# SEEDtk/kmers.anno

Hardware: AMD Instinct MI355X
Metric: kmer lookups/s + seqs annotated/s at 1/2/4/8 GPUs; achieved HBM GB/s vs roofline (higher is better)
Workload: dtype u64; 1 GPU; c5: 1M proteins per rank vs 10^8-entry multi-function signature table (HBM random access); proteins_per_gpu=1000000, windows_per_gpu=303576763, batch_windows=303576763, table_entries=100000000, functions=100000, k=8, min_hits=5, table_layout_m=6, table_minimizer_order=mod-sampling, table_placement=two-choice, parallelism=input-shard x1, table on this GPU

## Files before the change

kmers.anno_amd/csrc/kma_abi.cpp:

```cpp
#include <hip/hip_runtime.h>
#include <sched.h>

#include <algorithm>
#include <atomic>
#include <chrono>
#include <condition_variable>
#include <cstdarg>
#include <cstdio>
#include <cstdlib>
#include <cstring>
#include <memory>
#include <mutex>
#include <string>
#include <thread>
#include <vector>

#include "../../include/kmeranno.h"
#include "kma_distance.h"
#include "kma_hashanno.h"
#include "kma_internal.h"
#include "kma_pack.h"
#include "kma_tsv.h"

namespace {
// ... 1200 lines not shown
uint64_t contig_blocks(uint64_t n_bases) {
  return std::max<uint64_t>(1, (n_bases + kma::kContigTile - 1) / kma::kContigTile);
}

void codon_codes(const char* code, uint8_t out[64]) {
  for (int i = 0; i < 64; ++i)
    out[i] = (code[i] == '*' || code[i] == 'X') ? 0 : (uint8_t)(code[i] - 'A' + 1);
}

int contig_args(const kma_table* t, const Replica& r, kma_workspace* ws, const uint8_t* d_dna,
                const uint64_t* d_offsets, uint32_t n_contig, uint64_t n_bases, const char* code,
                uint32_t* d_tally, uint32_t n_fid, hipStream_t s, kma::ContigArgs* out) {
  kma::ContigArgs a{};
  a.slots = r.d_slots;
  a.n_buckets = (uint32_t)t->n_buckets;
  a.dna = d_dna;
  a.offsets = d_offsets;
  a.n_contig = n_contig;
  a.total_bases = n_bases;
  a.k = t->k;
  a.mlen = t->mlen;
  a.two_choice = t->two_choice ? 1u : 0u;
  a.staging = ws->d_cstage;
  a.block_counts = ws->d_ccounts;
  if (ws->cpending) KMA_HIP(hipMemsetAsync(ws->d_cprefix, 0, (ws->cgroups + 1) * 8, s));
  ws->cpending = true;
  a.group_sum = ws->d_cprefix;
  a.emit_done = reinterpret_cast<uint32_t*>(ws->d_cprefix + ws->cgroups);
  a.tally = d_tally;
  a.n_fid = d_tally ? n_fid : 0;
  codon_codes(code, a.codon_codes);
  *out = a;
  return KMA_OK;
}

int enqueue_contig_emit(kma_workspace* ws, kma::ContigArgs a, kma_hit* d_hits, uint64_t cap,
                        uint64_t* d_n_hits, hipStream_t s) {
  const uint64_t nb = contig_blocks(a.total_bases);
  a.out = d_hits;
  a.cap = d_hits ? cap : 0;
  a.n_hits = d_n_hits;
  KMA_HIP(kma::launch_contigs_emit(a, nb, s));
  ws->cpending = false;
  return KMA_OK;
}

struct PhaseClock {
  hipEvent_t* ev = nullptr;
  int n = 0;
  hipStream_t s = nullptr;
  PhaseClock(kma_workspace* ws, hipStream_t stream, const char* const* names, int n_phases)
      : s(stream) {
    if (!ws->timing) return;
    const uint32_t slot = ws->n_timed++ % kTimingRing;
    ev = &ws->events[kMaxEv * slot];
    ws->names[slot] = names;
    ws->n_phases[slot] = n_phases;
  }
  hipError_t mark() { return ev ? hipEventRecord(ev[n++], s) : hipSuccess; }
};

const char* const kDirectPhases[] = {"annotate_kernel"};
const char* const kPackedPhases[] = {"pack_kernel", "annotate_kernel"};
const char* const kContigPhases[] = {"contigs_probe_kernel", "scan_emit"};

uint32_t block_proteins(const kma_workspace* ws, uint32_t n_seq, uint64_t table_bytes) {
  const int64_t f = ws->opt_block_proteins != kOptUnset ? ws->opt_block_proteins
                                                         : opt(KMA_OPT_BLOCK_PROTEINS);
  if (f >= 1 && f <= kma::kBlockProteins) return (uint32_t)f;
  const uint64_t slots = (uint64_t)kma::kProteinOcc * (uint64_t)std::max(ws->n_cu, 1);
  return (uint64_t)n_seq / 6 > 4 * slots && table_bytes > kInfinityCacheBytes ? 6u : 4u;
}

uint32_t defer_below(const kma_workspace* ws, uint64_t n_groups) {
  const uint64_t slots = (uint64_t)kma::kProteinOcc * (uint64_t)std::max(ws->n_cu, 1);
  const int64_t f = ws->opt_defer != kOptUnset ? ws->opt_defer : opt(KMA_OPT_DEFER);
  if (f >= 0) return (uint32_t)std::min<int64_t>(64, f);
  return n_groups > slots && n_groups <= 4 * slots ? 3u : 0u;
}

enum class Input { kAscii, kPackOnDevice, kStream };

constexpr uint64_t kPackMinResidues = 1ull << 25;
bool pack_on_device(uint64_t n_residues) {
  const int64_t v = opt(KMA_OPT_PACKED_INPUT);
  return n_residues > 0 && (v == 2 || (v == 1 && n_residues >= kPackMinResidues));
}

int ensure_packed(const kma_workspace* ws) {
  if (ws->d_packed) return KMA_OK;
  return fail(KMA_E_CAPACITY, "workspace has no packed stream (kma_workspace_reserve_batch first)");
}

int annotate_proteins_on(const kma_table* t, const Replica& r, kma_workspace* ws,
                         const uint8_t* d_residues, const uint64_t* d_offsets, uint32_t n_seq,
                         uint64_t n_residues, int min_hits, uint32_t flags, int32_t* d_fid,
                         int32_t* d_count, uint8_t* d_status, uint32_t* d_tally, uint32_t n_fid,
                         hipStream_t s, Input input = Input::kAscii, uint64_t stream_first = 0) {
  kma::ProteinArgs a{};
  a.slots = r.d_slots;
  a.n_buckets = (uint32_t)t->n_buckets;
  a.lut = r.d_lut;
  a.residues = input == Input::kPackOnDevice ? ws->d_packed : d_residues;
  a.packed = input != Input::kAscii;
  a.stream_first = input == Input::kStream ? stream_first : 0;
  a.offsets = d_offsets;
  a.n_seq = n_seq;
  a.n_residues = (uint32_t)n_residues;
  a.k = t->k;
  a.mlen = t->mlen;
  a.two_choice = t->two_choice ? 1u : 0u;
  a.min_hits = min_hits;
  a.flags = flags;
  a.out_fid = d_fid;
  a.out_count = d_count;
  a.out_status = d_status;
  a.tally = d_tally;
  a.n_fid = d_tally ? n_fid : 0;
  a.gset = ws->d_gset;
  a.block_proteins = block_proteins(ws, n_seq, t->n_buckets * (uint64_t)kma::kBucketBytes);
  a.n_groups = (n_seq + a.block_proteins - 1) / a.block_proteins;
  a.defer_below = a.n_groups < (1u << 30) ? defer_below(ws, a.n_groups) : 0u;
  const bool pack = input == Input::kPackOnDevice;
  PhaseClock clk(ws, s, pack ? kPackedPhases : kDirectPhases, pack ? 2 : 1);
  KMA_HIP(clk.mark());
  if (pack) {
    KMA_HIP(kma::launch_pack_residues(d_residues, d_offsets, n_residues, r.d_lut, ws->d_packed,
                                      s));
    KMA_HIP(clk.mark());
  }
  KMA_HIP(kma::launch_annotate(a, s));
  KMA_HIP(clk.mark());
  return KMA_OK;
}

int check_protein_call(const kma_table* t, int min_hits, uint32_t flags) {
  if (!t) return fail(KMA_E_INVALID, "null table");
  if (kma::wide_k(t->k))
    return fail(KMA_E_INVALID, "the protein path takes tables of K <= 8 (this table: K = %d)",
                t->k);
  if (min_hits < 1) return fail(KMA_E_INVALID, "Min-hits must be positive.");
  if (flags & ~(KMA_F_END_EXCLUSIVE | KMA_F_MULTISET)) return fail(KMA_E_INVALID, "bad flags");
  return KMA_OK;
}

hipError_t stage_h2d(uint8_t* d_dst, uint8_t* h_pinned, const uint8_t* src, size_t len,
                     int device, hipStream_t s) {
  constexpr size_t kChunk = 2u << 20;
  const size_t n_chunks = (len + kChunk - 1) / kChunk;
  staging_pool().run(n_chunks, staging_threads(), [&](uint64_t i) {
    const size_t off = i * kChunk;
    std::memcpy(h_pinned + off, src + off, std::min(kChunk, len - off));
  });
  (void)device;
  return len ? hipMemcpyAsync(d_dst, h_pinned, len, hipMemcpyHostToDevice, s) : hipSuccess;
}

hipError_t stage_pack_h2d(uint8_t* d_stream, uint8_t* h_stream, const uint8_t* lut,
                          const uint8_t* residues, uint64_t n_res, uint64_t ga, uint64_t gb,
                          uint64_t tail, hipStream_t s) {
  constexpr uint64_t kChunkGroups = 1u << 15;
  const uint64_t n_chunks = std::max<uint64_t>(1, (gb - ga + kChunkGroups - 1) / kChunkGroups);
  staging_pool().run(n_chunks, staging_threads(), [&](uint64_t i) {
    const uint64_t g0 = ga + i * kChunkGroups, g1 = std::min(gb, g0 + kChunkGroups);
    const uint64_t r0 = 64 * g0, r1 = std::min(64 * g1, n_res);
    const uint64_t bytes = 40 * (g1 - g0) + (g1 == gb ? tail : 0);
    kma::pack_residues_host(lut, residues + r0, r1 > r0 ? r1 - r0 : 0, h_stream + 40 * g0, bytes);
  });
  const uint64_t bytes = 40 * (gb - ga) + tail;
// ... 318 lines not shown
    ws->names.assign(kTimingRing, nullptr);
    ws->n_phases.assign(kTimingRing, 0);
  }
  ws->timing = enable != 0;
  ws->n_timed = 0;
  return KMA_OK;
}

int kma_workspace_phases_read(kma_workspace* ws, uint32_t* n_calls, int* n_phases,
                              double* phase_ms, const char** phase_names) {
  if (!ws || !n_calls || !n_phases || !phase_ms) return fail(KMA_E_INVALID, "null argument");
  DeviceScope ds(ws->device);
  const uint32_t n = std::min(ws->n_timed, kTimingRing);
  *n_calls = 0;
  *n_phases = 0;
  for (int i = 0; i < KMA_MAX_PHASES; ++i) {
    phase_ms[i] = 0.0;
    if (phase_names) phase_names[i] = nullptr;
  }
  if (n == 0) return KMA_OK;
  const uint32_t last = (ws->n_timed - 1) % kTimingRing;
  const char* const* names = ws->names[last];
  const int np = ws->n_phases[last];
  for (uint32_t i = 0; i < n; ++i) {
    if (ws->names[i] != names) continue;
    hipEvent_t* e = &ws->events[kMaxEv * i];
    KMA_HIP(hipEventSynchronize(e[np]));
    for (int ph = 0; ph < np; ++ph) {
      float ms = 0;
      KMA_HIP(hipEventElapsedTime(&ms, e[ph], e[ph + 1]));
      phase_ms[ph] += ms;
    }
    ++*n_calls;
  }
  *n_phases = np;
  if (phase_names)
    for (int ph = 0; ph < np; ++ph) phase_names[ph] = names[ph];
  ws->n_timed = 0;
  return KMA_OK;
}

int kma_workspace_timing_read(kma_workspace* ws, uint32_t* n_calls, double* kernel_ms,
                              double* rest_ms) {
  if (!ws || !n_calls || !kernel_ms || !rest_ms) return fail(KMA_E_INVALID, "null argument");
  double ms[KMA_MAX_PHASES];
  const char* names[KMA_MAX_PHASES];
  int np = 0;
  if (int rc = kma_workspace_phases_read(ws, n_calls, &np, ms, names)) return rc;
  const bool contigs = np > 0 && names[0] == kContigPhases[0];
  *kernel_ms = 0;
  *rest_ms = 0;
  for (int ph = 0; ph < np; ++ph) (contigs && ph > 0 ? *rest_ms : *kernel_ms) += ms[ph];
  return KMA_OK;
}

int kma_workspace_destroy(kma_workspace* ws) {
  if (!ws) return KMA_OK;
  DeviceScope ds(ws->device);
  for (auto& e : ws->events) (void)hipEventDestroy(e);
  free_protein_scratch(ws);
  free_contig_scratch(ws);
  delete ws;
  return KMA_OK;
}

int kma_annotate_proteins_device(const kma_table* t, kma_workspace* ws, const uint8_t* d_residues,
                                 const uint64_t* d_offsets, uint32_t n_seq, uint64_t n_residues,
                                 int min_hits, uint32_t flags, int32_t* d_fid, int32_t* d_count,
                                 uint8_t* d_status, uint32_t* d_tally, uint32_t n_fid,
                                 void* stream) {
  if (int rc = check_protein_call(t, min_hits, flags)) return rc;
  if (!ws) return fail(KMA_E_INVALID, "null workspace");
  Replica rep;
  if (!replica_on(t, ws->device, &rep))
    return fail(KMA_E_INVALID, "table has no replica on the workspace's device %d", ws->device);
  const Replica* r = &rep;
  if (n_seq == 0) return KMA_OK;
  if (!d_residues || !d_offsets || !d_fid || !d_count || !d_status)
    return fail(KMA_E_INVALID, "null device buffer");
  if ((uintptr_t)d_residues & 7) return fail(KMA_E_INVALID, "residues must be 8-byte aligned");
  if (n_residues > ws->res_cap)
    return fail(KMA_E_CAPACITY, "workspace reserved for %llu residues, call needs %llu",
                (unsigned long long)ws->res_cap, (unsigned long long)n_residues);
  const bool pack = pack_on_device(n_residues);
  if (pack)
    if (int rc = ensure_packed(ws)) return rc;
  DeviceScope ds(r->device);
  if (ds.err != hipSuccess) return fail(KMA_E_DEVICE, "hipSetDevice(%d)", r->device);
  return annotate_proteins_on(t, *r, ws, d_residues, d_offsets, n_seq, n_residues, min_hits,
                              flags, d_fid, d_count, d_status, d_tally, n_fid,
                              static_cast<hipStream_t>(stream),
                              pack ? Input::kPackOnDevice : Input::kAscii);
}

uint64_t kma_packed_bytes(uint64_t n_residues) { return kma::packed_bytes(n_residues); }

int kma_pack_residues(const kma_table* t, const uint8_t* residues, uint64_t n, uint8_t* out,
                      uint64_t out_bytes) {
  if ((n && !residues) || !out) return fail(KMA_E_INVALID, "null argument");
  if (out_bytes < kma::packed_bytes(n))
    return fail(KMA_E_CAPACITY, "packed stream of %llu residues needs %llu bytes",
                (unsigned long long)n, (unsigned long long)kma::packed_bytes(n));
  uint8_t std_lut[256];
  if (!t) standard_lut(std_lut);
  const uint8_t* lut = t ? t->lut : std_lut;
  constexpr uint64_t kChunkGroups = 1u << 15;
  const uint64_t n_groups = (n + 63) / 64, n_chunks = (n_groups + kChunkGroups - 1) / kChunkGroups;
  if (n_chunks < 4) {
    kma::pack_residues_host(lut, residues, n, out, out_bytes);
    return KMA_OK;
  }
  staging_pool().run(n_chunks, staging_threads(), [&](uint64_t c) {
    const uint64_t g0 = c * kChunkGroups, g1 = std::min(n_groups, g0 + kChunkGroups);
    const uint64_t r0 = 64 * g0, r1 = std::min(64 * g1, n);
    const uint64_t bytes = g1 == n_groups ? out_bytes - 40 * g0 : 40 * (g1 - g0);
    kma::pack_residues_host(lut, residues + r0, r1 - r0, out + 40 * g0, bytes);
  });
  return KMA_OK;
}

int kma_annotate_packed_device(const kma_table* t, kma_workspace* ws, const uint8_t* d_stream,
                               const uint64_t* d_offsets, uint32_t n_seq, uint64_t n_residues,
                               int min_hits, uint32_t flags, int32_t* d_fid, int32_t* d_count,
                               uint8_t* d_status, uint32_t* d_tally, uint32_t n_fid,
                               void* stream) {
  if (int rc = check_protein_call(t, min_hits, flags)) return rc;
  if (!ws) return fail(KMA_E_INVALID, "null workspace");
  Replica rep;
  if (!replica_on(t, ws->device, &rep))
    return fail(KMA_E_INVALID, "table has no replica on the workspace's device %d", ws->device);
  if (n_seq == 0) return KMA_OK;
  if (!d_stream || !d_offsets || !d_fid || !d_count || !d_status)
    return fail(KMA_E_INVALID, "null device buffer");
  if ((uintptr_t)d_stream & 7) return fail(KMA_E_INVALID, "stream must be 8-byte aligned");
  if (n_residues > ws->res_cap)
    return fail(KMA_E_CAPACITY, "workspace reserved for %llu residues, call needs %llu",
                (unsigned long long)ws->res_cap, (unsigned long long)n_residues);
  DeviceScope ds(rep.device);
  if (ds.err != hipSuccess) return fail(KMA_E_DEVICE, "hipSetDevice(%d)", rep.device);
  return annotate_proteins_on(t, rep, ws, d_stream, d_offsets, n_seq, n_residues, min_hits, flags,
                              d_fid, d_count, d_status, d_tally, n_fid,
                              static_cast<hipStream_t>(stream), Input::kStream, 0);
}

int kma_annotate_proteins(const kma_table* tc, const uint8_t* residues, const uint64_t* offsets,
                          uint32_t n_seq, int min_hits, uint32_t flags, int32_t* out_fid,
                          int32_t* out_count, uint8_t* out_status, uint32_t* out_tally,
                          uint32_t n_fid) {
  if (int rc = check_protein_call(tc, min_hits, flags)) return rc;
  kma_table* t = const_cast<kma_table*>(tc);
  if (n_seq == 0) return KMA_OK;
  if (!residues || !offsets || !out_fid || !out_count || !out_status)
    return fail(KMA_E_INVALID, "null argument");
  if (const uint32_t s = offsets_decrease_at(offsets, n_seq); s < n_seq)
    return fail(KMA_E_INVALID, "offsets decrease at %u", s);
  const bool tally = out_tally && n_fid;
  const std::vector<Replica> reps = replicas(t);
  const int nr = (int)std::min<uint64_t>(reps.size(), n_seq);
  const std::vector<uint32_t> b = shard_bounds(offsets, n_seq, nr);
  std::vector<std::vector<uint32_t>> part(tally ? nr : 0, std::vector<uint32_t>(n_fid));
  const int64_t so = opt(KMA_OPT_HOST_SLICE);
  const uint64_t slice = so > 0 ? (uint64_t)so : 1ull << 31;
  const size_t width = staging_width(nr);
  const int rc = fan_out(nr, [&](int i) {
    ShardWidth sw(width);
    std::vector<uint32_t> st(tally ? n_fid : 0);
    for (uint32_t lo = b[i]; lo < b[i + 1];) {
// ... 793 lines not shown
```

kmers.anno_amd/csrc/kma_device.h:

```cpp
#pragma once

#include <hip/hip_runtime.h>
#include <stdint.h>

#include "kma_internal.h"

namespace kma {
namespace {

template <typename Op>
__device__ __forceinline__ uint32_t wave_reduce(uint32_t v, Op op) {
  v = op(v, (uint32_t)__builtin_amdgcn_mov_dpp((int)v, 0xB1, 0xF, 0xF, false));
  v = op(v, (uint32_t)__builtin_amdgcn_mov_dpp((int)v, 0x4E, 0xF, 0xF, false));
  v = op(v, (uint32_t)__builtin_amdgcn_mov_dpp((int)v, 0x141, 0xF, 0xF, false));
  v = op(v, (uint32_t)__builtin_amdgcn_mov_dpp((int)v, 0x140, 0xF, 0xF, false));
  const uint32_t r0 = (uint32_t)__builtin_amdgcn_readlane((int)v, 0);
  const uint32_t r1 = (uint32_t)__builtin_amdgcn_readlane((int)v, 16);
  const uint32_t r2 = (uint32_t)__builtin_amdgcn_readlane((int)v, 32);
  const uint32_t r3 = (uint32_t)__builtin_amdgcn_readlane((int)v, 48);
  return op(op(r0, r1), op(r2, r3));
}
__device__ __forceinline__ uint32_t wave_max(uint32_t v) {
  return wave_reduce(v, [](uint32_t x, uint32_t y) { return x > y ? x : y; });
}
__device__ __forceinline__ uint32_t wave_sum(uint32_t v) {
  return wave_reduce(v, [](uint32_t x, uint32_t y) { return x + y; });
}
__device__ __forceinline__ uint32_t popc_below(uint64_t m) {
  return __builtin_amdgcn_mbcnt_hi((uint32_t)(m >> 32),
                                   __builtin_amdgcn_mbcnt_lo((uint32_t)m, 0u));
}

__device__ __forceinline__ uint64_t funnel(uint64_t lo, uint64_t hi, uint32_t sh) {
  return sh ? ((lo >> sh) | (hi << (64u - sh))) : lo;
}
__device__ __forceinline__ uint64_t window_bytes(const uint8_t* __restrict__ res, uint64_t pos) {
  const uint64_t* src = reinterpret_cast<const uint64_t*>(res + (pos & ~7ull));
  return funnel(src[0], src[1], (uint32_t)(pos & 7) * 8u);
}
struct WinWords {
  uint64_t lo, hi;
  uint32_t sh;
};
__device__ __forceinline__ WinWords window_words(const uint8_t* __restrict__ res, uint64_t pos) {
  const uint64_t* src = reinterpret_cast<const uint64_t*>(res + (pos & ~7ull));
  return WinWords{src[0], src[1], (uint32_t)(pos & 7) * 8u};
}
__device__ __forceinline__ uint64_t win_bytes(const WinWords& w) { return funnel(w.lo, w.hi, w.sh); }

__device__ __forceinline__ WinWords window_words_packed(const uint8_t* __restrict__ stream,
                                                        uint64_t j) {
  const uint64_t bit = 5 * j, byte = bit >> 3;
  const uint64_t* src = reinterpret_cast<const uint64_t*>(stream + (byte & ~7ull));
  return WinWords{src[0], src[1], (uint32_t)(((byte & 7) << 3) | (bit & 7))};
}
__device__ __forceinline__ uint64_t bswap64(uint64_t v) {
  const uint32_t lo = (uint32_t)v, hi = (uint32_t)(v >> 32);
  const uint32_t slo = __builtin_amdgcn_perm(0u, lo, 0x00010203u);
  const uint32_t shi = __builtin_amdgcn_perm(0u, hi, 0x00010203u);
  return (uint64_t)slo << 32 | shi;
}
template <int K>
__device__ __forceinline__ uint64_t packed_key(const WinWords& w) {
  const uint64_t be = bswap64(funnel(w.lo, w.hi, w.sh & 56u));
  return (be << (w.sh & 7u)) >> (64 - 5 * K);
}

template <int K>
__device__ __forceinline__ bool pack_window(const uint8_t* lut, uint64_t bytes, uint64_t& key) {
  uint32_t c[K];
#pragma unroll
  for (int j = 0; j < K; ++j) c[j] = lut[(uint32_t)(bytes >> (8 * j)) & 0xFFu];
  uint64_t v = 0;
  bool ok = true;
#pragma unroll
  for (int j = 0; j < K; ++j) {
    ok = ok && c[j] != 0u;
    v = (v << 5) | c[j];
  }
  key = v;
  return ok;
}

constexpr int kBucketQuads = kBucketBytes / 16;
__device__ __forceinline__ void scan_half(const uint4 (&q)[4], int half, uint64_t key, bool& hit,
                                          bool& empty, uint32_t& fid, uint32_t& slot) {
  const uint32_t klo = (uint32_t)key, khi = (uint32_t)(key >> 32) << 24;
  const uint32_t lo[8] = {q[0].x, q[0].z, q[1].x, q[1].z, q[2].x, q[2].z, q[3].x, q[3].z};
  const uint32_t hi[8] = {q[0].y, q[0].w, q[1].y, q[1].w, q[2].y, q[2].w, q[3].y, q[3].w};
#pragma unroll
  for (int j = 0; j < 8; ++j) {
    const bool m = lo[j] == klo && (hi[j] & kKeyHiMask) == khi;
    fid = m ? (hi[j] & kFidMask) : fid;
    slot = m ? (uint32_t)(8 * half + j) : slot;
    hit = hit || m;
    empty = empty || lo[j] == 0u;
  }
}

#ifndef KMA_WALK_GROUP
#define KMA_WALK_GROUP 1
#endif
constexpr int kWalkGroup = KMA_WALK_GROUP;
__device__ __forceinline__ bool walk_chain(const uint64_t* __restrict__ slots, uint32_t n_buckets,
                                           uint32_t b, uint64_t key, uint32_t& fid,
                                           uint32_t& sid, bool two_choice = false,
                                           uint32_t* walked = nullptr) {
  if (two_choice) {
    const uint32_t ab = alt_bucket(key, b, n_buckets);
    const uint4* bp = reinterpret_cast<const uint4*>(slots + (uint64_t)ab * kSlotsPerBucket);
    uint4 q[kBucketQuads];
#pragma unroll
    for (int i = 0; i < kBucketQuads; ++i) q[i] = bp[i];
    bool h = false, e = false;
    uint32_t slot = 0;
#pragma unroll
    for (int half = 0; half < kBucketHalves; ++half) {
      const uint4 part[4] = {q[4 * half], q[4 * half + 1], q[4 * half + 2], q[4 * half + 3]};
      scan_half(part, half, key, h, e, fid, slot);
    }
    sid = ab * kSlotsPerBucket + slot;
    if (walked) *walked = 1;
    return h;
  }
  bool hit = false, empty = false;
  const uint32_t home = b;
  uint32_t slot = 0, steps = 1;
  while (!hit && !empty && steps < n_buckets) {
    uint32_t bb[kWalkGroup];
    uint4 q[kWalkGroup][kBucketQuads];
#pragma unroll
    for (int g = 0; g < kWalkGroup; ++g) {
      const uint32_t i = steps + g;
      b = chain_bucket(home, i < n_buckets ? i : 0u, n_buckets);
      bb[g] = b;
      const uint4* bp = reinterpret_cast<const uint4*>(slots + (uint64_t)b * kSlotsPerBucket);
#pragma unroll
      for (int i = 0; i < kBucketQuads; ++i) q[g][i] = bp[i];
    }
#pragma unroll
    for (int g = 0; g < kWalkGroup; ++g) {
      if (hit || empty || steps >= n_buckets) break;
      bool h = false, e = false;
#pragma unroll
      for (int half = 0; half < kBucketHalves; ++half) {
        const uint4 part[4] = {q[g][4 * half], q[g][4 * half + 1], q[g][4 * half + 2],
                               q[g][4 * half + 3]};
        scan_half(part, half, key, h, e, fid, slot);
      }
      hit = h;
      empty = e;
      sid = bb[g] * kSlotsPerBucket + slot;
      ++steps;
    }
  }
  if (walked) *walked = steps - 1;
  return hit;
}

template <int R>
__device__ __forceinline__ uint32_t quad_bcast(uint32_t v) {
  return (uint32_t)__builtin_amdgcn_mov_dpp((int)v, R * 0x55, 0xF, 0xF, false);
}
__device__ __forceinline__ uint32_t quad_or(uint32_t v) {
// ... 134 lines not shown
```

kmers.anno_amd/csrc/kma_kernels.hip:

```cpp
#include <cstring>
#include <rocprim/rocprim.hpp>

#include <algorithm>
#include <cstdio>
#include <cstdlib>

#include "../../include/kmeranno.h"
#include "kma_internal.h"
#include "kma_device.h"


namespace kma {
namespace {


template <bool Wide>
__global__ __launch_bounds__(256) void build_insert_kernel(uint64_t* slots, uint32_t* winner,
                                                           uint32_t n_buckets, int k, int m,
                                                           const uint64_t* __restrict__ keys,
                                                           uint64_t n, uint32_t* status) {
  constexpr int S = Wide ? kWideSlots : kSlotsPerBucket;
  for (uint64_t i = blockIdx.x * (uint64_t)blockDim.x + threadIdx.x; i < n;
       i += (uint64_t)gridDim.x * blockDim.x) {
    const uint64_t key = keys[i];
// ... 192 lines not shown
        if (chosen >> j & 1ull) continue;
        const uint64_t key = skeys[ids[i + j]];
        const uint32_t mask = filter_need<S>((uint32_t)key);
        const bool alt_full = load && load[alt_bucket(key, h, n_buckets)] >= S;
        const uint32_t fresh = (uint32_t)__popc(mask & ~set) + (alt_full ? 32u : 0u);
        if (fresh < best_new) {
          best = j;
          best_new = fresh;
          best_mask = mask;
          if (fresh == 0) break;
        }
      }
      chosen |= 1ull << best;
      set |= best_mask;
      away[ids[i + best]] = 1;
    }
  }
}

__global__ __launch_bounds__(256) void build_two_choice_filter_kernel(uint64_t* slots,
                                                                      uint32_t n_buckets, int k,
                                                                      int m, uint32_t* stats) {
  constexpr int S = kSlotsPerBucket;
  const uint64_t n_slots = (uint64_t)n_buckets * S;
  uint32_t entries = 0, displaced = 0;
  for (uint64_t i = blockIdx.x * (uint64_t)blockDim.x + threadIdx.x; i < n_slots;
       i += (uint64_t)gridDim.x * blockDim.x) {
    const uint64_t v = __hip_atomic_load(slots + i, __ATOMIC_RELAXED, __HIP_MEMORY_SCOPE_AGENT);
    if ((uint32_t)v == 0u) continue;
    const uint64_t key = slot_key(v);
    const uint32_t b = (uint32_t)(i / S), h = home_bucket(key, k, m, n_buckets);
    entries++;
    if (b != h) {
      displaced++;
      for (int f = 0; f < kFilterBits; ++f) {
        const uint32_t pos = filter_pos<S>((uint32_t)key, f);
        uint32_t* meta = reinterpret_cast<uint32_t*>(slots + (uint64_t)h * S + pos / kFilterBits) + 1;
        const uint32_t bit = 1u << (kFidBits + pos % kFilterBits);
        if (!(__hip_atomic_load(meta, __ATOMIC_RELAXED, __HIP_MEMORY_SCOPE_AGENT) & bit))
          atomicOr(meta, bit);
      }
    }
  }
  entries = wave_sum(entries);
  displaced = wave_sum(displaced);
  if ((threadIdx.x & 63) == 0) {
    if (entries) atomicAdd(stats + 0, entries);
    atomicMax(stats + 1, displaced ? 2u : entries ? 1u : 0u);
    if (displaced) atomicAdd(stats + 2, displaced);
  }
}


#ifdef KMA_BLOCK_CLOCK
__device__ uint64_t g_block_clk[8 * 65536];
#define KMA_CLK_SET(i, v)                                          \
  do {                                                             \
    if (threadIdx.x == 0 && blockIdx.x < 65535)                    \
      g_block_clk[8 * blockIdx.x + (i)] = (v);                     \
  } while (0)
#define KMA_CLK(i) KMA_CLK_SET(i, wall_clock64())
#define KMA_CLK_HW()                                                \
  KMA_CLK_SET(6, (uint64_t)__builtin_amdgcn_s_getreg(20 | (15 << 11)) << 32 | \
                     (uint32_t)__builtin_amdgcn_s_getreg(4 | (31 << 11)))
#else
#define KMA_CLK_SET(i, v) ((void)0)
#define KMA_CLK(i) ((void)0)
#define KMA_CLK_HW() ((void)0)
#endif

#ifdef KMA_TUNE_COUNT
__device__ unsigned long long g_walk_stats[8];
#define KMA_COUNT(i, v)                                                                    \
  do {                                                                                     \
    const unsigned long long kma_v_ = (unsigned long long)(v);   \
    if ((threadIdx.x & 63) == 0)                                                           \
      __hip_atomic_fetch_add(&g_walk_stats[i], kma_v_, __ATOMIC_RELAXED,                   \
                             __HIP_MEMORY_SCOPE_AGENT);                                    \
  } while (0)
#else
#define KMA_COUNT(i, v) ((void)0)
#endif

template <int P>
struct ProteinSmem {
  __attribute__((aligned(16))) uint32_t pool[kSetPool];
  uint32_t chain_q[kWavesPerBlock][2 * kChainQ];
  uint32_t pbeg[P + 1];
  uint32_t pwin[P];
  uint32_t pset[P];
  uint32_t pcap[P];
  uint32_t pmin[P], pmax[P], pcnt[P];
  uint32_t plist[P];
  uint32_t skip;
  uint8_t lut[256];
};
static_assert(sizeof(ProteinSmem<kBlockProteins>) <= 163840 / kProteinOcc,
              "protein-path LDS must leave kProteinOcc blocks per CU");

__device__ __forceinline__ bool lds_set_insert(uint32_t* set, uint32_t cap, uint32_t key) {
  uint32_t i = set_slot(key, cap);
  for (;;) {
    const uint32_t o = atomicCAS(set + i, 0u, key);
    if (o == 0u) return true;
    if (o == key) return false;
    i = i + 1 == cap ? 0u : i + 1;
  }
}
__device__ __forceinline__ bool global_set_insert(uint32_t* set, uint32_t cap, uint32_t key) {
  uint32_t i = set_slot(key, cap);
  for (;;) {
    uint32_t o = 0u;
    __hip_atomic_compare_exchange_strong(set + i, &o, key, __ATOMIC_RELAXED, __ATOMIC_RELAXED,
                                         __HIP_MEMORY_SCOPE_AGENT);
    if (o == 0u) return true;
    if (o == key) return false;
    i = i + 1 == cap ? 0u : i + 1;
  }
}

template <int P>
__device__ __forceinline__ void record_hit(ProteinSmem<P>& sm, const ProteinArgs& a,
                                           uint64_t span_lo, bool multiset, uint32_t p,
                                           uint32_t fid, uint32_t sid) {
  atomicMin(&sm.pmin[p], fid);
  atomicMax(&sm.pmax[p], fid);
  bool fresh = true;
#ifdef KMA_TUNE_NO_SET
  fresh = false;
  if (false) {
#else
  if (!multiset) {
#endif
    const uint32_t base = sm.pset[p];
    if (base != kGlobalSet) {
      fresh = lds_set_insert(sm.pool + base, sm.pcap[p], sid + 1u);
    } else {
      a.gset[2 * (span_lo + sm.pbeg[p]) + atomicAdd(&sm.plist[p], 1u)] = sid + 1u;
      fresh = false;
    }
  }
  if (fresh) atomicAdd(&sm.pcnt[p], 1u);
}

template <int P>
__device__ __forceinline__ void dedupe_lists(ProteinSmem<P>& sm, const ProteinArgs& a,
                                             uint64_t span_lo) {
  const int t = threadIdx.x;
  for (int p = 0; p < P; ++p) {
    if (sm.pset[p] != kGlobalSet) continue;
    const uint32_t h = sm.plist[p], b0 = sm.pbeg[p];
    if (h == 0) continue;
    const uint32_t* list = a.gset + 2 * (span_lo + b0);
    uint32_t fresh = 0;
    if (h < (uint32_t)kSetPool) {
      uint4* pool4 = reinterpret_cast<uint4*>(sm.pool);
      for (uint32_t i = t; i < (uint32_t)kSetPool / 4; i += 256) pool4[i] = make_uint4(0u, 0u, 0u, 0u);
      __syncthreads();
      for (uint32_t i = t; i < h; i += 256) fresh += lds_set_insert(sm.pool, kSetPool, list[i]);
    } else {
      const uint32_t L = sm.pbeg[p + 1] - b0;
      uint32_t* set = a.gset + 2 * (span_lo + b0) + L;
      for (uint32_t i = t; i < L; i += 256)
        __hip_atomic_store(set + i, 0u, __ATOMIC_RELAXED, __HIP_MEMORY_SCOPE_AGENT);
      __threadfence();
      __syncthreads();
      for (uint32_t i = t; i < h; i += 256) fresh += global_set_insert(set, L, list[i]);
    }
    fresh = wave_sum(fresh);
    if ((t & 63) == 0 && fresh) atomicAdd(&sm.pcnt[p], fresh);
    __syncthreads();
  }
}

template <int P>
__device__ __forceinline__ uint32_t protein_at(const uint32_t (&pb)[P + 1], uint32_t x) {
  uint32_t p = 0;
#pragma unroll
  for (int i = 1; i < P; ++i) p += x >= pb[i] ? 1u : 0u;
  return p;
}
template <int P>
__device__ __forceinline__ bool window_at(const uint32_t (&pe)[P], uint32_t x, uint32_t p) {
  uint32_t ended = 0;
#pragma unroll
  for (int i = 0; i < P; ++i) ended += x >= pe[i] ? 1u : 0u;
  return ended == p;
}

__device__ __forceinline__ uint32_t lane_window(int t) {
#if KMA_LANE_PERM
  return (uint32_t)((t >> 6) * 64 + 16 * (t & 3) + ((t & 63) >> 2));
#else
  return (uint32_t)t;
#endif
}

#ifndef KMA_XCD_GROUPS
#define KMA_XCD_GROUPS 1
#endif
__device__ __forceinline__ uint32_t xcd_group(uint32_t b, uint32_t n) {
#if KMA_XCD_GROUPS
  const uint32_t per = n >> 3;
  return b < 8u * per ? (b & 7u) * per + (b >> 3) : b;
#else
  (void)n;
  return b;
#endif
}

struct GroupHead {
  uint32_t p0, np;
  uint64_t beg_raw;
  uint64_t span_lo;
};
__device__ __forceinline__ void head_offsets(const ProteinArgs& a, uint32_t g, GroupHead& h) {
  const int lane = threadIdx.x & 63, wave = threadIdx.x >> 6;
  h.p0 = g * a.block_proteins;
  h.np = min(a.block_proteins, a.n_seq - h.p0);
  h.beg_raw = wave == 0 && lane <= (int)h.np ? a.offsets[h.p0 + lane] : 0u;
  h.span_lo = a.offsets[h.p0] - a.offsets[0];
}
template <bool Packed>
__device__ __forceinline__ const uint8_t* head_res(const ProteinArgs& a, const GroupHead& h,
                                                   uint64_t& pos0) {
  if (Packed) {
    pos0 = a.stream_first + h.span_lo;
    return a.residues;
  }
  const uint8_t* res0 = a.residues + a.offsets[0] + h.span_lo;
  pos0 = (uintptr_t)res0 & 7u;
  return res0 - pos0;
}
template <bool Packed>
__device__ __forceinline__ WinWords load_win(const uint8_t* __restrict__ res, uint64_t pos) {
  return Packed ? window_words_packed(res, pos) : window_words(res, pos);
}
template <int U, bool Packed>
__device__ __forceinline__ void head_residues(const ProteinArgs& a, const GroupHead& h,
                                              uint32_t tw, WinWords (&ww)[U]) {
  uint64_t pos0;
  const uint8_t* res = head_res<Packed>(a, h, pos0);
  const uint64_t lim = a.n_residues - h.span_lo;
#pragma unroll
  for (int j = 0; j < U; ++j) {
    const uint32_t x = j * 256u + tw;
    ww[j] = load_win<Packed>(res, (x < lim ? x : 0u) + pos0);
  }
}

template <int K, int M, int P, bool Packed>
__device__ __forceinline__ void annotate_block(const ProteinArgs& a, ProteinSmem<P>& sm,
                                               const GroupHead& h, WinWords (&ww)[kProbeWin],
                                               const int pass = -1) {
  constexpr int U = kProbeWin;
  const int t = threadIdx.x, lane = t & 63, wave = t >> 6, part = t & 3;
  const bool multiset = (a.flags & KMA_F_MULTISET) != 0;
  const uint32_t tw = lane_window(t);
  const uint32_t p0 = h.p0, np = h.np;
  const uint64_t beg_raw = h.beg_raw, span_lo = h.span_lo;
  const uint64_t o0 = a.offsets[0];
  uint64_t pos0;
  const uint8_t* __restrict__ res = head_res<Packed>(a, h, pos0);
  if (wave == 0) {
    const uint64_t beg = lane <= (int)np ? beg_raw - o0 : 0u;
    const uint64_t end = __shfl_down(beg, 1, 64);
    const uint64_t lo = __shfl(beg, 0, 64), span_end = __shfl(beg, (int)np, 64);
    if (pass >= 0 && lane == 0) {
      const bool short_group = span_end - lo < (uint64_t)a.defer_below * 256u * kProbeWin;
      sm.skip = short_group != (pass == 1) ? 1u : 0u;
    }
    if (lane <= P) sm.pbeg[lane] = (uint32_t)((lane <= (int)np ? beg : span_end) - lo);
    if (lane < P) {
      uint32_t nw = 0;
      if (lane < (int)np) {
        const int64_t n = (int64_t)(end - beg) - K + ((a.flags & KMA_F_END_EXCLUSIVE) ? 0 : 1);
        nw = n > 0 ? (uint32_t)n : 0u;
      }
      sm.pwin[lane] = nw;
      sm.pcap[lane] = (nw == 0 || multiset) ? 0u : ((nw + (nw >> 1) + 4u) & ~3u);
      sm.pmin[lane] = 0xFFFFFFFFu;
      sm.pmax[lane] = 0u;
      sm.pcnt[lane] = 0u;
      sm.plist[lane] = 0u;
    }
    __builtin_amdgcn_wave_barrier();
    if (lane == 0) {
      uint32_t sum = 0;
      for (int p = 0; p < P; ++p) sum += sm.pcap[p];
      uint32_t top = 0;
      if (sum <= (uint32_t)kSetPool) {
        for (int p = 0; p < P; ++p) {
          sm.pset[p] = top;
          top += sm.pcap[p];
        }
      } else {
        uint32_t done = 0;
        for (int it = 0; it < P; ++it) {
          int best = -1;
          for (int p = 0; p < P; ++p)
            if (!(done >> p & 1u) && (best < 0 || sm.pcap[p] > sm.pcap[best])) best = p;
          done |= 1u << best;
          const uint32_t cap = sm.pcap[best];
          const bool fits = top + cap <= (uint32_t)kSetPool;
          sm.pset[best] = fits ? top : kGlobalSet;
          top += fits ? cap : 0u;
        }
      }
      sm.chain_q[0][0] = top;
    }
  }
  __syncthreads();
  if (pass >= 0 && sm.skip) return;
  const uint32_t used = sm.chain_q[0][0];
  uint32_t pb[P + 1], pe[P];
#pragma unroll
  for (int i = 0; i <= P; ++i) pb[i] = __builtin_amdgcn_readfirstlane(sm.pbeg[i]);
#pragma unroll
  for (int i = 0; i < P; ++i) pe[i] = __builtin_amdgcn_readfirstlane(sm.pbeg[i] + sm.pwin[i]);
  const uint32_t span = pb[P];
  __syncthreads();
  uint4* pool4 = reinterpret_cast<uint4*>(sm.pool);
  KMA_CLK(1);
  for (uint32_t i = t; i < used / 4; i += 256) pool4[i] = make_uint4(0u, 0u, 0u, 0u);
  __syncthreads();

  const uint64_t* __restrict__ slots = a.slots;
  const uint32_t nb = a.n_buckets;
  const bool two_choice = a.two_choice != 0;
  const uint8_t* lut = sm.lut;
  uint32_t* cq = sm.chain_q[wave];
  uint32_t cn = 0;
  constexpr uint32_t stride = 256u * U;
  auto chain_flush = [&]() {
    __builtin_amdgcn_wave_barrier();
    KMA_COUNT(0, 1);
    KMA_COUNT(1, cn);
#ifdef KMA_TUNE_COUNT
    uint32_t wsum = 0, wmax = 0;
#endif
    for (uint32_t e = lane; e < cn; e += 64) {
      const uint32_t w2 = cq[2 * e + 1];
      const uint64_t key = (uint64_t)(w2 & 0xFFu) << 32 | cq[2 * e];
      const uint32_t p = w2 >> 8;
      uint32_t fid = 0, sid = 0;
#ifdef KMA_TUNE_COUNT
      uint32_t walked = 0;
      const bool hit = walk_chain(slots, nb, home_bucket(key, K, M, nb), key, fid, sid, two_choice,
                                  &walked);
#else
      const bool hit = walk_chain(slots, nb, home_bucket(key, K, M, nb), key, fid, sid, two_choice);
#endif
      if (hit) record_hit<P>(sm, a, span_lo, multiset, p, fid, sid);
#ifdef KMA_TUNE_COUNT
      {
        const uint32_t s1 = chain_bucket(home_bucket(key, K, M, nb), 1u, nb);
        const bool first = hit && sid / kSlotsPerBucket == s1;
        KMA_COUNT(4, __popcll(__ballot(hit)));
        KMA_COUNT(5, __popcll(__ballot(first)));
        wsum += walked;
        wmax = walked > wmax ? walked : wmax;
      }
#endif
    }
#ifdef KMA_TUNE_COUNT
    KMA_COUNT(6, wave_sum(wsum));
    KMA_COUNT(7, wave_max(wmax));
#endif
    __builtin_amdgcn_wave_barrier();
    cn = 0;
  };
  struct Prep {
    uint32_t klo[U], khi[U], need[U], bk[U];
  };
  auto prep = [&](uint32_t xs, Prep& o) {
#pragma unroll
    for (int j = 0; j < U; ++j) {
      const uint32_t x = xs + j * 256u + tw;
      const uint32_t p = protein_at<P>(pb, x);
      uint64_t key;
      bool ok;
      if (Packed) {
        key = packed_key<K>(ww[j]);
        ok = key != 0 && x < span && window_at<P>(pe, x, p);
      } else {
        ok = pack_window<K>(lut, win_bytes(ww[j]), key) && x < span && window_at<P>(pe, x, p);
      }
      o.klo[j] = (uint32_t)key;
      o.khi[j] = (uint32_t)(key >> 32) << 24 | (ok ? 0u : 1u);
      o.need[j] = filter_need<kSlotsPerBucket>(o.klo[j]);
      o.bk[j] = p << kBucketBits | (ok ? home_bucket(key, K, M, nb) : 0u);
    }
  };
  auto gather = [&](const Prep& c, uint4 (&q)[U][4][kBucketHalves]) {
#pragma unroll
    for (int j = 0; j < U; ++j) {
      const uint32_t b0 = quad_bcast<0>(c.bk[j]), b1 = quad_bcast<1>(c.bk[j]);
      const uint32_t b2 = quad_bcast<2>(c.bk[j]), b3 = quad_bcast<3>(c.bk[j]);
      const uint32_t bb[4] = {b0, b1, b2, b3};
#pragma unroll
      for (int r = 0; r < 4; ++r) {
        const uint4* bp = reinterpret_cast<const uint4*>(slots) + part +
                          (uint64_t)(bb[r] & kBucketIdx) * kBucketQuads;
#pragma unroll
        for (int h = 0; h < kBucketHalves; ++h) q[j][r][h] = bp[4 * h];
      }
    }
  };
  auto load_residues = [&](uint32_t xs) {
#pragma unroll
    for (int j = 0; j < U; ++j) {
      const uint32_t x = xs + j * 256u + tw;
      ww[j] = load_win<Packed>(res, (x < span ? x : 0u) + pos0);
    }
  };
  auto settle = [&](uint32_t x0, const Prep& c, const uint4 (&q)[U][4][kBucketHalves]) {
    uint32_t word[U];
#pragma unroll
    for (int j = 0; j < U; ++j) {
      word[j] = 0;
      uint32_t raw[4];
      (void)raw;
#pragma unroll
      for (int r = 0; r < 4; ++r) {
        const uint32_t kl = r == 0 ? quad_bcast<0>(c.klo[j]) : r == 1 ? quad_bcast<1>(c.klo[j])
                          : r == 2 ? quad_bcast<2>(c.klo[j]) : quad_bcast<3>(c.klo[j]);
        const uint32_t kh = r == 0 ? quad_bcast<0>(c.khi[j]) : r == 1 ? quad_bcast<1>(c.khi[j])
                          : r == 2 ? quad_bcast<2>(c.khi[j]) : quad_bcast<3>(c.khi[j]);
        const uint32_t nd = r == 0 ? quad_bcast<0>(c.need[j]) : r == 1 ? quad_bcast<1>(c.need[j])
                          : r == 2 ? quad_bcast<2>(c.need[j]) : quad_bcast<3>(c.need[j]);
#if KMA_QUAD_XPOSE
        raw[r] = match_part_raw(q[j][r], kl, kh, nd, part);
#else
        const uint32_t v = match_part(q[j][r], kl, kh, nd, part);
        word[j] = part == r ? v : word[j];
#endif
      }
#if KMA_QUAD_XPOSE
      word[j] = quad_reduce_scatter(raw, part);
#endif
    }
#pragma unroll
    for (int j = 0; j < U; ++j) {
      const bool probed = (c.khi[j] & 1u) == 0u;
      const uint32_t w = probed ? word[j] : 0u;
#ifdef KMA_TUNE_COUNT
      KMA_COUNT(2, __popcll(__ballot(probed)));
      KMA_COUNT(3, __popcll(__ballot((w & kWordHit) != 0u)));
#endif
      if (w & kWordHit)
        record_hit<P>(sm, a, span_lo, multiset, c.bk[j] >> kBucketBits, w & kFidMask,
                      (c.bk[j] & kBucketIdx) * kSlotsPerBucket + ((w >> kSlotShift) & kSlotMask));
#ifdef KMA_TUNE_NO_WALK
      const bool pend = false;
#else
      const bool pend = probed && w == 0u;
#endif
      const uint64_t m = __ballot(pend);
      if (pend) {
        const uint32_t e = cn + popc_below(m);
        cq[2 * e] = c.klo[j];
        cq[2 * e + 1] = (c.khi[j] >> 24) | (c.bk[j] >> kBucketBits) << 8;
      }
      cn += (uint32_t)__popcll(m);
    }
    if (cn > (uint32_t)(kChainQ - 64 * U)) chain_flush();
  };
  for (uint32_t x0 = 0; x0 < span; x0 += stride) {
    Prep cur;
    prep(x0, cur);
    uint4 q[U][4][kBucketHalves];
    gather(cur, q);
    load_residues(x0 + stride);
    settle(x0, cur, q);
    if (x0 == 0) KMA_CLK(2);
  }
  KMA_CLK(3);
  KMA_CLK_SET(7, (span + stride - 1) / stride);
  if (cn) chain_flush();
  KMA_CLK(4);
  __syncthreads();
  if (!multiset) dedupe_lists<P>(sm, a, span_lo);
  if (t < (int)np) {
    const uint32_t mn = sm.pmin[t], mx = sm.pmax[t], cnt = sm.pcnt[t];
    int32_t fid_out = -1, cnt_out = 0;
    uint8_t st;
    if (mn == 0xFFFFFFFFu) {
      st = KMA_STATUS_NONE;
    } else if (mn != mx) {
      st = KMA_STATUS_AMBIGUOUS;
    } else {
      fid_out = (int32_t)mn;
      cnt_out = (int32_t)cnt;
      st = cnt >= (uint32_t)a.min_hits ? KMA_STATUS_CALLED : KMA_STATUS_BELOW_MIN;
      if (st == KMA_STATUS_CALLED && a.tally && mn < a.n_fid) atomicAdd(a.tally + mn, 1u);
    }
    a.out_fid[p0 + t] = fid_out;
    a.out_count[p0 + t] = cnt_out;
    a.out_status[p0 + t] = st;
  }
}

template <int K, int M, bool Packed>
constexpr int protein_occ() {
  return (M == 0 && (Packed || K < 8)) || (!Packed && (M & kOrderMod)) ? 6 : kProteinOcc;
}
template <int K, int M, int P, bool Packed>
__global__ __launch_bounds__(256) __attribute__((amdgpu_waves_per_eu(protein_occ<K, M, Packed>(), 8))) void annotate_kernel(
    ProteinArgs a) {
  __shared__ ProteinSmem<P> sm;
  KMA_CLK(0);
  const int t = threadIdx.x;
  const uint8_t lut_b = Packed ? 0 : a.lut[t];
  const bool second = a.defer_below && blockIdx.x >= a.n_groups;
  GroupHead h;
  WinWords ww[kProbeWin];
  const uint32_t b = blockIdx.x - (second ? a.n_groups : 0u);
  head_offsets(a, a.defer_below ? b : xcd_group(b, a.n_groups), h);
  head_residues<kProbeWin, Packed>(a, h, lane_window(t), ww);
  if (!Packed) sm.lut[t] = lut_b;
  annotate_block<K, M, P, Packed>(a, sm, h, ww, a.defer_below ? (second ? 1 : 0) : -1);
  KMA_CLK(5);
  KMA_CLK_HW();
}

#ifdef KMA_TUNE_COUNT
}
}
extern "C" int kma_debug_walk_stats(uint64_t* out, int reset) {
  hipError_t e = hipMemcpyFromSymbol(out, HIP_SYMBOL(kma::g_walk_stats), 64, 0,
                                     hipMemcpyDeviceToHost);
  if (e == hipSuccess && reset) {
    const uint64_t z[8] = {};
    e = hipMemcpyToSymbol(HIP_SYMBOL(kma::g_walk_stats), z, 64, 0, hipMemcpyHostToDevice);
  }
  return (int)e;
}
namespace kma {
namespace {
#endif

#ifdef KMA_BLOCK_CLOCK
}
}
extern "C" int kma_debug_block_clock(uint64_t* out, uint64_t n) {
  return (int)hipMemcpyFromSymbol(out, HIP_SYMBOL(kma::g_block_clk), 8 * n, 0,
                                  hipMemcpyDeviceToHost);
}
namespace kma {
namespace {
#endif

__device__ __forceinline__ uint32_t contig_of(const uint64_t* __restrict__ off, uint32_t n,
                                              uint64_t g) {
  uint32_t lo = 0, hi = n;
  while (hi - lo > 1) {
    const uint32_t mid = (lo + hi) >> 1;
    if (off[mid] <= g) lo = mid; else hi = mid;
  }
  return lo;
}

__device__ __forceinline__ uint32_t base2(uint8_t c) {
  switch (c | 0x20) {
    case 't': case 'u': return 0u;
    case 'c': return 1u;
    case 'a': return 2u;
    case 'g': return 3u;
    default: return 4u;
  }
}


constexpr int kOffCache = 64;

__device__ __forceinline__ uint32_t contig_of_wave(const uint64_t* __restrict__ off, uint32_t n,
                                                   uint64_t g) {
  const uint32_t lane = threadIdx.x & 63;
  uint32_t lo = 0, span = n;
  while (span > 1) {
    const uint32_t step = (span + 63) / 64;
    const uint32_t c = lo + lane * step;
    const bool le = lane * step < span && off[c] <= g;
    const uint32_t k = (uint32_t)__popcll(__ballot(le)) - 1u;
    const uint32_t nlo = lo + k * step;
    span = min(step, lo + span - nlo);
    lo = nlo;
  }
  return lo;
}

#ifndef KMA_CONTIG_OCC
#define KMA_CONTIG_OCC (KMA_CONTIG_SEQ > 1 ? 7 : 8)
#endif
template <int K, int M>
__global__ __launch_bounds__(256) __attribute__((amdgpu_waves_per_eu(KMA_CONTIG_OCC, 8))) void contigs_probe_quad_kernel(
    ContigArgs a) {
  constexpr bool kWide = wide_k(K);
  constexpr int kS = kWide ? kWideSlots : kSlotsPerBucket;
  constexpr int kQ = kWide ? 4 : kBucketQuads;
  constexpr int kH = kWide ? 1 : kBucketHalves;
  constexpr int kSpan = kContigTile + 3 * K;
  __shared__ uint8_t bases[kSpan];
  __shared__ uint8_t aa_p[kSpan], aa_m[kSpan];
// ... 710 lines not shown
```

Before: 111.3 billion kmer lookups/s.

## Stage ASCII residues through LDS as packed 5-bit words; skip device packing for big tables

The ASCII kernel path no longer has every lane load two overlapping 8-byte words per window and translate K bytes through the LUT. A subset of lanes loads contiguous residue words once, converts them to the 5-bit packed form in an LDS staging buffer, and each lane then reads its window from that buffer with the packed-key extractor. The LDS set pool shrinks to make room for the buffer, and the occupancy hint for mod-order ASCII kernels is raised. Device-side packing is also turned off by default when the table exceeds Infinity Cache, so this workload now takes the staged ASCII path instead of the packing pre-pass.

Result: no change. 110.4 billion kmer lookups/s (-0.8%).

```diff
diff --git a/kmers.anno_amd/csrc/kma_abi.cpp b/kmers.anno_amd/csrc/kma_abi.cpp
--- a/kmers.anno_amd/csrc/kma_abi.cpp
+++ b/kmers.anno_amd/csrc/kma_abi.cpp
@@ -1306,9 +1306,10 @@
 enum class Input { kAscii, kPackOnDevice, kStream };
 
 constexpr uint64_t kPackMinResidues = 1ull << 25;
-bool pack_on_device(uint64_t n_residues) {
+bool pack_on_device(uint64_t n_residues, uint64_t table_bytes) {
   const int64_t v = opt(KMA_OPT_PACKED_INPUT);
-  return n_residues > 0 && (v == 2 || (v == 1 && n_residues >= kPackMinResidues));
+  return n_residues > 0 && (v == 2 || (v == 1 && n_residues >= kPackMinResidues &&
+                                       table_bytes <= kInfinityCacheBytes));
 }
 
 int ensure_packed(const kma_workspace* ws) {
@@ -1793,7 +1794,7 @@
   if (n_residues > ws->res_cap)
     return fail(KMA_E_CAPACITY, "workspace reserved for %llu residues, call needs %llu",
                 (unsigned long long)ws->res_cap, (unsigned long long)n_residues);
-  const bool pack = pack_on_device(n_residues);
+  const bool pack = pack_on_device(n_residues, t->n_buckets * (uint64_t)kma::kBucketBytes);
   if (pack)
     if (int rc = ensure_packed(ws)) return rc;
   DeviceScope ds(r->device);
diff --git a/kmers.anno_amd/csrc/kma_device.h b/kmers.anno_amd/csrc/kma_device.h
--- a/kmers.anno_amd/csrc/kma_device.h
+++ b/kmers.anno_amd/csrc/kma_device.h
@@ -42,11 +42,6 @@
   uint64_t lo, hi;
   uint32_t sh;
 };
-__device__ __forceinline__ WinWords window_words(const uint8_t* __restrict__ res, uint64_t pos) {
-  const uint64_t* src = reinterpret_cast<const uint64_t*>(res + (pos & ~7ull));
-  return WinWords{src[0], src[1], (uint32_t)(pos & 7) * 8u};
-}
-__device__ __forceinline__ uint64_t win_bytes(const WinWords& w) { return funnel(w.lo, w.hi, w.sh); }
 
 __device__ __forceinline__ WinWords window_words_packed(const uint8_t* __restrict__ stream,
                                                         uint64_t j) {
@@ -64,22 +59,6 @@
 __device__ __forceinline__ uint64_t packed_key(const WinWords& w) {
   const uint64_t be = bswap64(funnel(w.lo, w.hi, w.sh & 56u));
   return (be << (w.sh & 7u)) >> (64 - 5 * K);
-}
-
-template <int K>
-__device__ __forceinline__ bool pack_window(const uint8_t* lut, uint64_t bytes, uint64_t& key) {
-  uint32_t c[K];
-#pragma unroll
-  for (int j = 0; j < K; ++j) c[j] = lut[(uint32_t)(bytes >> (8 * j)) & 0xFFu];
-  uint64_t v = 0;
-  bool ok = true;
-#pragma unroll
-  for (int j = 0; j < K; ++j) {
-    ok = ok && c[j] != 0u;
-    v = (v << 5) | c[j];
-  }
-  key = v;
-  return ok;
 }
 
 constexpr int kBucketQuads = kBucketBytes / 16;
diff --git a/kmers.anno_amd/csrc/kma_kernels.hip b/kmers.anno_amd/csrc/kma_kernels.hip
--- a/kmers.anno_amd/csrc/kma_kernels.hip
+++ b/kmers.anno_amd/csrc/kma_kernels.hip
@@ -298,9 +298,21 @@
 #define KMA_COUNT(i, v) ((void)0)
 #endif
 
-template <int P>
-struct ProteinSmem {
-  __attribute__((aligned(16))) uint32_t pool[kSetPool];
+constexpr int kStageWords = 10;
+constexpr int kStageBytes = 56;
+constexpr int kStagePool = 32;
+static_assert(5 * kStageWords <= kStageBytes && kStageBytes % 8 == 0, "staging buffer size");
+template <bool Staged>
+struct StageBuf {};
+template <>
+struct StageBuf<true> {
+  __attribute__((aligned(8))) uint8_t stage[kWavesPerBlock][kProbeWin][kStageBytes];
+};
+template <int P, bool Staged>
+struct ProteinSmem : StageBuf<Staged> {
+  static constexpr int kP = P;
+  static constexpr int kPool = kSetPool - (Staged ? kStagePool : 0);
+  __attribute__((aligned(16))) uint32_t pool[kPool];
   uint32_t chain_q[kWavesPerBlock][2 * kChainQ];
   uint32_t pbeg[P + 1];
   uint32_t pwin[P];
@@ -311,7 +323,8 @@
   uint32_t skip;
   uint8_t lut[256];
 };
-static_assert(sizeof(ProteinSmem<kBlockProteins>) <= 163840 / kProteinOcc,
+static_assert(sizeof(ProteinSmem<kBlockProteins, false>) <= 163840 / kProteinOcc &&
+                  sizeof(ProteinSmem<kBlockProteins, true>) <= 163840 / kProteinOcc,
               "protein-path LDS must leave kProteinOcc blocks per CU");
 
 __device__ __forceinline__ bool lds_set_insert(uint32_t* set, uint32_t cap, uint32_t key) {
@@ -335,8 +348,8 @@
   }
 }
 
-template <int P>
-__device__ __forceinline__ void record_hit(ProteinSmem<P>& sm, const ProteinArgs& a,
+template <class Smem>
+__device__ __forceinline__ void record_hit(Smem& sm, const ProteinArgs& a,
                                            uint64_t span_lo, bool multiset, uint32_t p,
                                            uint32_t fid, uint32_t sid) {
   atomicMin(&sm.pmin[p], fid);
@@ -359,9 +372,10 @@
   if (fresh) atomicAdd(&sm.pcnt[p], 1u);
 }
 
-template <int P>
-__device__ __forceinline__ void dedupe_lists(ProteinSmem<P>& sm, const ProteinArgs& a,
-                                             uint64_t span_lo) {
+template <class Smem>
+__device__ __forceinline__ void dedupe_lists(Smem& sm, const ProteinArgs& a, uint64_t span_lo) {
+  constexpr int P = Smem::kP;
+  constexpr uint32_t kPool = Smem::kPool;
   const int t = threadIdx.x;
   for (int p = 0; p < P; ++p) {
     if (sm.pset[p] != kGlobalSet) continue;
@@ -369,11 +383,11 @@
     if (h == 0) continue;
     const uint32_t* list = a.gset + 2 * (span_lo + b0);
     uint32_t fresh = 0;
-    if (h < (uint32_t)kSetPool) {
+    if (h < kPool) {
       uint4* pool4 = reinterpret_cast<uint4*>(sm.pool);
-      for (uint32_t i = t; i < (uint32_t)kSetPool / 4; i += 256) pool4[i] = make_uint4(0u, 0u, 0u, 0u);
+      for (uint32_t i = t; i < kPool / 4; i += 256) pool4[i] = make_uint4(0u, 0u, 0u, 0u);
       __syncthreads();
-      for (uint32_t i = t; i < h; i += 256) fresh += lds_set_insert(sm.pool, kSetPool, list[i]);
+      for (uint32_t i = t; i < h; i += 256) fresh += lds_set_insert(sm.pool, kPool, list[i]);
     } else {
       const uint32_t L = sm.pbeg[p + 1] - b0;
       uint32_t* set = a.gset + 2 * (span_lo + b0) + L;
@@ -448,27 +462,61 @@
   pos0 = (uintptr_t)res0 & 7u;
   return res0 - pos0;
 }
-template <bool Packed>
-__device__ __forceinline__ WinWords load_win(const uint8_t* __restrict__ res, uint64_t pos) {
-  return Packed ? window_words_packed(res, pos) : window_words(res, pos);
-}
-template <int U, bool Packed>
+template <int U>
 __device__ __forceinline__ void head_residues(const ProteinArgs& a, const GroupHead& h,
                                               uint32_t tw, WinWords (&ww)[U]) {
   uint64_t pos0;
-  const uint8_t* res = head_res<Packed>(a, h, pos0);
+  const uint8_t* res = head_res<true>(a, h, pos0);
   const uint64_t lim = a.n_residues - h.span_lo;
 #pragma unroll
   for (int j = 0; j < U; ++j) {
     const uint32_t x = j * 256u + tw;
-    ww[j] = load_win<Packed>(res, (x < lim ? x : 0u) + pos0);
-  }
+    ww[j] = window_words_packed(res, (x < lim ? x : 0u) + pos0);
+  }
+}
+
+__device__ __forceinline__ bool stage_lane(int lane) {
+  return lane < 16 * kProbeWin && (lane & 15) < kStageWords;
+}
+__device__ __forceinline__ uint64_t stage_load(const uint8_t* __restrict__ res, uint32_t pos0,
+                                               uint32_t xs, uint32_t lim, int lane, int wave) {
+  uint32_t s = xs + (uint32_t)(lane >> 4) * 256u + (uint32_t)wave * 64u;
+  s = s < lim ? s : 0u;
+  const uint32_t last = (uint32_t)(((uint64_t)lim + pos0 + 32u) >> 3) - 1u;
+  const uint32_t wi = min(s / 8u + (uint32_t)(lane & 15), last);
+  return reinterpret_cast<const uint64_t*>(res)[wi];
+}
+template <class Smem>
+__device__ __forceinline__ void stage_store(Smem& sm, uint64_t sw, int lane, int wave) {
+  if (stage_lane(lane)) {
+    const uint8_t* lut = sm.lut;
+    const uint32_t lo = (uint32_t)sw, hi = (uint32_t)(sw >> 32);
+    const uint32_t c0 = lut[lo & 0xFFu], c1 = lut[(lo >> 8) & 0xFFu];
+    const uint32_t c2 = lut[(lo >> 16) & 0xFFu], c3 = lut[lo >> 24];
+    const uint32_t c4 = lut[hi & 0xFFu], c5 = lut[(hi >> 8) & 0xFFu];
+    const uint32_t c6 = lut[(hi >> 16) & 0xFFu], c7 = lut[hi >> 24];
+    const uint32_t top = c0 << 3 | c1 >> 2;
+    const uint32_t low = c1 << 30 | c2 << 25 | c3 << 20 | c4 << 15 | c5 << 10 | c6 << 5 | c7;
+    uint8_t* d = sm.stage[wave][lane >> 4] + 5 * (lane & 15);
+    d[0] = (uint8_t)top;
+    d[1] = (uint8_t)(low >> 24);
+    d[2] = (uint8_t)(low >> 16);
+    d[3] = (uint8_t)(low >> 8);
+    d[4] = (uint8_t)low;
+  }
+  __builtin_amdgcn_wave_barrier();
+}
+__device__ __forceinline__ WinWords stage_window(const uint8_t* buf, uint32_t r) {
+  const uint32_t bit = 5u * r, byte = bit >> 3;
+  const uint64_t* src = reinterpret_cast<const uint64_t*>(buf + (byte & ~7u));
+  return WinWords{src[0], src[1], ((byte & 7u) << 3) | (bit & 7u)};
 }
 
 template <int K, int M, int P, bool Packed>
-__device__ __forceinline__ void annotate_block(const ProteinArgs& a, ProteinSmem<P>& sm,
+__device__ __forceinline__ void annotate_block(const ProteinArgs& a, ProteinSmem<P, !Packed>& sm,
                                                const GroupHead& h, WinWords (&ww)[kProbeWin],
-                                               const int pass = -1) {
+                                               uint64_t& sw, const int pass = -1) {
+  using Smem = ProteinSmem<P, !Packed>;
   constexpr int U = kProbeWin;
   const int t = threadIdx.x, lane = t & 63, wave = t >> 6, part = t & 3;
   const bool multiset = (a.flags & KMA_F_MULTISET) != 0;
@@ -505,7 +553,7 @@
       uint32_t sum = 0;
       for (int p = 0; p < P; ++p) sum += sm.pcap[p];
       uint32_t top = 0;
-      if (sum <= (uint32_t)kSetPool) {
+      if (sum <= (uint32_t)Smem::kPool) {
         for (int p = 0; p < P; ++p) {
           sm.pset[p] = top;
           top += sm.pcap[p];
@@ -518,7 +566,7 @@
             if (!(done >> p & 1u) && (best < 0 || sm.pcap[p] > sm.pcap[best])) best = p;
           done |= 1u << best;
           const uint32_t cap = sm.pcap[best];
-          const bool fits = top + cap <= (uint32_t)kSetPool;
+          const bool fits = top + cap <= (uint32_t)Smem::kPool;
           sm.pset[best] = fits ? top : kGlobalSet;
           top += fits ? cap : 0u;
         }
@@ -544,7 +592,6 @@
   const uint64_t* __restrict__ slots = a.slots;
   const uint32_t nb = a.n_buckets;
   const bool two_choice = a.two_choice != 0;
-  const uint8_t* lut = sm.lut;
   uint32_t* cq = sm.chain_q[wave];
   uint32_t cn = 0;
   constexpr uint32_t stride = 256u * U;
@@ -567,7 +614,7 @@
 #else
       const bool hit = walk_chain(slots, nb, home_bucket(key, K, M, nb), key, fid, sid, two_choice);
 #endif
-      if (hit) record_hit<P>(sm, a, span_lo, multiset, p, fid, sid);
+      if (hit) record_hit(sm, a, span_lo, multiset, p, fid, sid);
 #ifdef KMA_TUNE_COUNT
       {
         const uint32_t s1 = chain_bucket(home_bucket(key, K, M, nb), 1u, nb);
@@ -595,13 +642,11 @@
       const uint32_t x = xs + j * 256u + tw;
       const uint32_t p = protein_at<P>(pb, x);
       uint64_t key;
-      bool ok;
-      if (Packed) {
+      if constexpr (Packed)
         key = packed_key<K>(ww[j]);
-        ok = key != 0 && x < span && window_at<P>(pe, x, p);
-      } else {
-        ok = pack_window<K>(lut, win_bytes(ww[j]), key) && x < span && window_at<P>(pe, x, p);
-      }
+      else
+        key = packed_key<K>(stage_window(sm.stage[wave][j], (uint32_t)pos0 + (tw & 63u)));
+      const bool ok = key != 0 && x < span && window_at<P>(pe, x, p);
       o.klo[j] = (uint32_t)key;
       o.khi[j] = (uint32_t)(key >> 32) << 24 | (ok ? 0u : 1u);
       o.need[j] = filter_need<kSlotsPerBucket>(o.klo[j]);
@@ -624,10 +669,14 @@
     }
   };
   auto load_residues = [&](uint32_t xs) {
-#pragma unroll
-    for (int j = 0; j < U; ++j) {
-      const uint32_t x = xs + j * 256u + tw;
-      ww[j] = load_win<Packed>(res, (x < span ? x : 0u) + pos0);
+    if constexpr (Packed) {
+#pragma unroll
+      for (int j = 0; j < U; ++j) {
+        const uint32_t x = xs + j * 256u + tw;
+        ww[j] = window_words_packed(res, (x < span ? x : 0u) + pos0);
+      }
+    } else {
+      if (stage_lane(lane)) sw = stage_load(res, (uint32_t)pos0, xs, span, lane, wave);
     }
   };
   auto settle = [&](uint32_t x0, const Prep& c, const uint4 (&q)[U][4][kBucketHalves]) {
@@ -665,7 +714,7 @@
       KMA_COUNT(3, __popcll(__ballot((w & kWordHit) != 0u)));
 #endif
       if (w & kWordHit)
-        record_hit<P>(sm, a, span_lo, multiset, c.bk[j] >> kBucketBits, w & kFidMask,
+        record_hit(sm, a, span_lo, multiset, c.bk[j] >> kBucketBits, w & kFidMask,
                       (c.bk[j] & kBucketIdx) * kSlotsPerBucket + ((w >> kSlotShift) & kSlotMask));
 #ifdef KMA_TUNE_NO_WALK
       const bool pend = false;
@@ -683,6 +732,7 @@
     if (cn > (uint32_t)(kChainQ - 64 * U)) chain_flush();
   };
   for (uint32_t x0 = 0; x0 < span; x0 += stride) {
+    if constexpr (!Packed) stage_store(sm, sw, lane, wave);
     Prep cur;
     prep(x0, cur);
     uint4 q[U][4][kBucketHalves];
@@ -696,7 +746,7 @@
   if (cn) chain_flush();
   KMA_CLK(4);
   __syncthreads();
-  if (!multiset) dedupe_lists<P>(sm, a, span_lo);
+  if (!multiset) dedupe_lists(sm, a, span_lo);
   if (t < (int)np) {
     const uint32_t mn = sm.pmin[t], mx = sm.pmax[t], cnt = sm.pcnt[t];
     int32_t fid_out = -1, cnt_out = 0;
@@ -719,23 +769,31 @@
 
 template <int K, int M, bool Packed>
 constexpr int protein_occ() {
-  return (M == 0 && (Packed || K < 8)) || (!Packed && (M & kOrderMod)) ? 6 : kProteinOcc;
+  return M == 0 && (Packed || K < 8) ? 6 : kProteinOcc;
 }
 template <int K, int M, int P, bool Packed>
 __global__ __launch_bounds__(256) __attribute__((amdgpu_waves_per_eu(protein_occ<K, M, Packed>(), 8))) void annotate_kernel(
     ProteinArgs a) {
-  __shared__ ProteinSmem<P> sm;
+  __shared__ ProteinSmem<P, !Packed> sm;
   KMA_CLK(0);
   const int t = threadIdx.x;
   const uint8_t lut_b = Packed ? 0 : a.lut[t];
   const bool second = a.defer_below && blockIdx.x >= a.n_groups;
   GroupHead h;
   WinWords ww[kProbeWin];
+  uint64_t sw = 0;
   const uint32_t b = blockIdx.x - (second ? a.n_groups : 0u);
   head_offsets(a, a.defer_below ? b : xcd_group(b, a.n_groups), h);
-  head_residues<kProbeWin, Packed>(a, h, lane_window(t), ww);
-  if (!Packed) sm.lut[t] = lut_b;
-  annotate_block<K, M, P, Packed>(a, sm, h, ww, a.defer_below ? (second ? 1 : 0) : -1);
+  if constexpr (Packed) {
+    head_residues<kProbeWin>(a, h, lane_window(t), ww);
+  } else {
+    uint64_t pos0;
+    const uint8_t* res = head_res<Packed>(a, h, pos0);
+    if (stage_lane(t & 63))
+      sw = stage_load(res, (uint32_t)pos0, 0u, a.n_residues - (uint32_t)h.span_lo, t & 63, t >> 6);
+    sm.lut[t] = lut_b;
+  }
+  annotate_block<K, M, P, Packed>(a, sm, h, ww, sw, a.defer_below ? (second ? 1 : 0) : -1);
   KMA_CLK(5);
   KMA_CLK_HW();
 }
```
